# adobe/3D-FM-GAN

Hardware: AMD Instinct MI355X
Metric: (photo,render) pairs/sec (higher is better)
Workload: dtype f32; 1 GPU; pairs1024: cfg4 shard: E_Tsr+E_W+E_W_Plus(18 styles) on 256^2 -> co-mod -> Generator(1024) forward, fp32, B=8/GPU; pairs_per_gpu=8, global_pairs=8, image_size=1024, parallelism=replicas x1 (batch-sharded, no collective), launch=eager, ranks=1, full=False

## Files before the change

### 3d-fm-gan_amd/op/_native.py

```python
import ctypes
import os

import torch

_HERE = os.path.dirname(os.path.abspath(__file__))
LIB_PATH = os.environ.get('FMGAN_LIB') or os.path.join(os.path.dirname(_HERE), 'csrc', 'libfmgan_hip.so')

F32, F64, F16 = 0, 1, 2
FMGAN_OK, FMGAN_EUNSUPPORTED = 0, -2
LPIPS_SIZE = 256
_DTYPES = {torch.float32: F32, torch.float64: F64, torch.float16: F16}

_lib = None

amp_fwd = torch.amp.custom_fwd(device_type='cuda', cast_inputs=torch.float32)
amp_bwd = torch.amp.custom_bwd(device_type='cuda')


def _sig(fn, argtypes, restype=ctypes.c_int):
    fn.argtypes = argtypes
    fn.restype = restype
    return fn


def lib():
    global _lib
    if _lib is not None:
        return _lib
    if not os.path.exists(LIB_PATH):
        raise RuntimeError(
            f'{LIB_PATH} not found: the HIP extension is not built. Run `make -C {os.path.dirname(LIB_PATH)}` '
            f'(or __graft_entry__.build()). There is no CPU or PyTorch fallback for these ops.')
    L = ctypes.CDLL(LIB_PATH)
    vp, i, f, ll = ctypes.c_void_p, ctypes.c_int, ctypes.c_float, ctypes.c_longlong
    _sig(L.fmgan_abi_version, [])
    _sig(L.fmgan_status_string, [i], ctypes.c_char_p)
    _sig(L.fmgan_upfirdn2d_select, [i] * 15)
    _sig(L.fmgan_upfirdn2d_out_size, [i] * 12 + [ctypes.POINTER(i)] * 2)
    _sig(L.fmgan_upfirdn2d, [i, vp, vp, vp] + [i] * 15 + [vp])
    _sig(L.fmgan_upfirdn2d_strided, [i, vp, vp, vp] + [i] * 4 + [ll, i] + [i] * 11 + [vp])
    _sig(L.fmgan_blur_noise_bias_act_f32, [vp] * 3 + [i] * 4 + [ll, i] + [i] * 6 + [vp] * 3 + [i, f, f, vp])
    _sig(L.fmgan_blur_noise_bias_act_select, [vp] * 3 + [i] * 4 + [ll, i] + [i] * 6)
    _sig(L.fmgan_blur_noise_bias_act_path_f32, [vp] * 3 + [i] * 4 + [ll, i] + [i] * 6 + [vp] * 3 + [i, f, f, i, vp])
    _sig(L.fmgan_fused_bias_act, [i, vp, vp, vp, vp, ll, i, i, i, i, f, f, vp])
    _sig(L.fmgan_noise_bias_act_f32, [vp] * 5 + [i] * 4 + [f, f, vp])
    _sig(L.fmgan_fused_bias_act_bwd_blocks, [ll, i])
    _sig(L.fmgan_fused_bias_act_bwd_f32, [vp] * 4 + [ll, i, f, f, vp])
    _sig(L.fmgan_prelu_backward_blocks, [ll, i])
    _sig(L.fmgan_prelu_backward_f32, [vp] * 5 + [ll, i, vp])
    _sig(L.fmgan_face_region_blocks, [i, ll])
    _sig(L.fmgan_face_region_loss_f32, [vp] * 3 + [i, i, ll, vp])
    _sig(L.fmgan_face_region_backward_f32, [vp] * 4 + [i, i, ll, vp])
    _sig(L.fmgan_render_mask_f32, [vp] * 2 + [i, i, ll, vp])
    _sig(L.fmgan_face_input_blocks, [i] * 4)
    _sig(L.fmgan_face_input_f32, [vp] * 5 + [i] * 4 + [vp])
    _sig(L.fmgan_lpips_pair_input_select, [i] * 8)
    _sig(L.fmgan_lpips_pair_input_f32, [vp] * 5 + [i] * 8 + [vp])
    _sig(L.fmgan_projection_loss_select, [i] * 4)
    _sig(L.fmgan_projection_loss_blocks, [i] * 4)
    _sig(L.fmgan_projection_loss_fwd_f32, [vp] * 7 + [i] * 4 + [vp])
    _sig(L.fmgan_projection_loss_bwd_f32, [vp] * 7 + [i] * 4 + [vp])
    _sig(L.fmgan_fid_stats_select, [i] * 2)
    _sig(L.fmgan_fid_stats_update_f32, [vp] * 4 + [i, i, vp])
    _sig(L.fmgan_fid_stats_finish_f64, [vp] * 3 + [ll, vp, vp, i, vp])
    _sig(L.fmgan_inception_input_select, [i] * 3)
    _sig(L.fmgan_inception_input_f32, [vp, vp] + [i] * 4 + [vp])
    _sig(L.fmgan_lpips_distance_blocks, [i] * 3)
    _sig(L.fmgan_lpips_distance_f32, [vp] * 4 + [i, i, i, f, vp])
    _sig(L.fmgan_lpips_distance_backward_f32, [vp] * 6 + [i, i, i, f, vp])
    _sig(L.fmgan_bn_prelu_f32, [vp] * 5 + [f, vp, vp] + [vp] * 4 + [f, vp, vp] + [i] * 5 + [vp])
    _sig(L.fmgan_se_pool_chunks, [i] * 4)
    _sig(L.fmgan_se_pool_f32, [vp, vp] + [i] * 4 + [vp])
    _sig(L.fmgan_se_gate_f32, [vp, i, ll] + [vp] * 4 + [f] + [vp] * 3 + [i] * 3 + [vp])
    _sig(L.fmgan_ir_tail_f32, [vp] * 5 + [f, vp, vp] + [i] * 3 + [vp] * 4 + [f, vp] + [vp] * 4 + [f, vp] + [i] * 4 + [vp])
    _sig(L.fmgan_modconv_demod_f32, [vp] * 3 + [i] * 4 + [f, f, vp])
    _sig(L.fmgan_modconv_wsq_f32, [vp] * 2 + [i] * 3 + [vp])
    _sig(L.fmgan_modconv_demod_wsq_f32, [vp] * 3 + [i] * 3 + [f, f, vp])
    _sig(L.fmgan_equal_linear_f32, [vp] * 4 + [i] * 3 + [vp])
    _sig(L.fmgan_wino_weight_f32, [vp, vp, i, i, vp])
    _sig(L.fmgan_wino_input_f32, [vp] * 3 + [i] * 4 + [vp])
    _sig(L.fmgan_wino_output_f32, [vp] * 6 + [i] * 6 + [f, f, vp])
    _sig(L.fmgan_modconv_weight_prep_f32, [vp, vp, i, i, i, f, i, vp])
    _sig(L.fmgan_modconv2d_workspace_bytes, [i] * 6, ll)
    _sig(L.fmgan_modconv2d_f32, [vp] * 5 + [i] * 6 + [vp] * 3 + [i, i, f, f, ll, i, vp, ll, vp])
    _sig(L.fmgan_modconv_weight_bf16_bytes, [i] * 3, ll)
    _sig(L.fmgan_modconv_weight_to_bf16, [vp, vp, i, i, i, vp])
    _sig(L.fmgan_modconv2d_bf16_supported, [i] * 6)
    _sig(L.fmgan_modconv2d_bf16, [vp] * 5 + [i] * 6 + [vp] * 3 + [i, i, f, f, ll, i, vp])
    _sig(L.fmgan_modconv_weight_bf16x3_bytes, [i] * 3, ll)
    _sig(L.fmgan_modconv_weight_to_bf16x3, [vp, vp, i, i, i, vp])
    _sig(L.fmgan_modconv2d_bf16x3_supported, [i] * 6)
    _sig(L.fmgan_modconv2d_bf16x3, [vp] * 5 + [i] * 6 + [vp] * 3 + [i, i, f, f, ll, i, vp])
    _sig(L.fmgan_modconv2d_rgb_fusable, [i] * 5)
    _sig(L.fmgan_modconv2d_select, [i] * 8 + [ctypes.POINTER(i)] * 5)
    _sig(L.fmgan_modconv2d_tiles, [ctypes.POINTER(i), i])
    _sig(L.fmgan_torgb_weight_mod_f32, [vp] * 3 + [i] * 3 + [f, vp])
    _sig(L.fmgan_modconv2d_rgb_f32, [vp] * 5 + [i] * 5 + [vp] * 3 + [i, i, f, f] + [vp] * 4 + [i, vp])
    _sig(L.fmgan_modconv_wgrad_workspace_bytes, [i] * 5, ll)
    _sig(L.fmgan_modconv_wgrad_f32, [vp] * 5 + [i] * 5 + [f, vp, ll, vp])
    _sig(L.fmgan_modconv_wgrad_mode_workspace_bytes, [i] * 6, ll)
    _sig(L.fmgan_modconv_wgrad_mode_f32, [vp] * 5 + [i] * 6 + [f, vp, ll, vp])
    _sig(L.fmgan_images_to_tensor, [vp, vp, i, i, i, f, f, vp])
    _sig(L.fmgan_resize_output_size, [i, i, i, ctypes.POINTER(ctypes.c_int), ctypes.POINTER(ctypes.c_int)])
    _sig(L.fmgan_resize_plan_ints, [i] * 4, ll)
    _sig(L.fmgan_resize_plan, [i] * 4 + [vp, ll])
    _sig(L.fmgan_resize_bilinear_u8, [vp] * 4 + [i] * 5 + [f, f, vp])
    _sig(L.fmgan_tensor_to_images, [vp, vp, i, i, i, f, f, vp])
    _sig(L.fmgan_torgb_f32, [vp] * 6 + [i] * 4 + [f, vp])
    _sig(L.fmgan_torgb_backward_splits, [i] * 3)
    _sig(L.fmgan_torgb_backward_f32, [vp] * 6 + [i] * 4 + [f, vp])
    _sig(L.fmgan_refresh_entry_bytes, [])
    _sig(L.fmgan_weight_refresh_blocks, [i, i, i, i, ll], ll)
    _sig(L.fmgan_weight_refresh_f32, [vp, i, ll, vp])
    _sig(L.fmgan_style_bank_entry_bytes, [])
    _sig(L.fmgan_style_bank_f32, [vp, i, vp, vp, i, i, i, vp, vp])
    _sig(L.fmgan_demod_bank_f32, [vp, i, vp, i, vp, vp])
    if L.fmgan_abi_version() != 1:
        raise RuntimeError('libfmgan_hip.so ABI version mismatch')
    _lib = L
    return L


def check(status, what):
    if status != FMGAN_OK:
        raise RuntimeError(f'{what}: {lib().fmgan_status_string(status).decode()} (status {status})')


def served(status, what):
    if status == FMGAN_EUNSUPPORTED:
        return False
    check(status, what)
    return True


def require_gpu(t, name):
    if not t.is_cuda:
        raise RuntimeError(f'{name} must be a CUDA tensor (this build has no CPU path)')


def dtype_code(t):
    try:
        return _DTYPES[t.dtype]
    except KeyError:
        raise RuntimeError(f'unsupported dtype {t.dtype}: float32/float64/float16 only') from None


def ptr(t):
    return None if t is None else t.data_ptr()


def fp(t):
    if t is None:
        return None
    if t.dtype != torch.float32 or not t.is_cuda:
        raise RuntimeError(f'libfmgan_hip f32 entry point got a {t.dtype} tensor on {t.device}: float32 GPU tensors only '
                           f'(cast before the call; under autocast the package\'s autograd Functions do)')
    return t.data_ptr()


def require_f32_gpu(what, named, contiguous=True, same_device=True):
    first = None
    for t, name in named:
        if t is None:
            continue
        require_gpu(t, name)
        fp(t)
        if contiguous and not t.is_contiguous():
            raise RuntimeError(f'{what}: {name} must be contiguous, got strides {t.stride()}')
        if first is None:
            first = (t.device, name)
        elif same_device and t.device != first[0]:
            raise RuntimeError(f'{what}: {name} must be on {first[1]}\'s device')


class on_device:

    def __init__(self, t):
        self.dev = t.device
        self.guard = None

    def __enter__(self):
        if torch.cuda.current_device() != self.dev.index:
            self.guard = torch.cuda.device(self.dev)
            self.guard.__enter__()
        return torch.cuda.current_stream(self.dev).cuda_stream

    def __exit__(self, *exc):
        if self.guard is not None:
            self.guard.__exit__(*exc)
        return False


BLUR_PATHS = {}


class _NullObserver:
    wants_paths = False

    def begin(self, name, info):
        return None

    def end(self, token):
        pass


_observer = _NullObserver()


def set_observer(obs=None):
    global _observer
    _observer = obs if obs is not None else _NullObserver()


class launching(on_device):

    def __init__(self, t, name, info):
        on_device.__init__(self, t)
        self.name, self.info = name, info

    def __enter__(self):
        stream = on_device.__enter__(self)
        self.tok = _observer.begin(self.name, self.info)
        return stream

    def __exit__(self, *exc):
        if exc[0] is None:
            _observer.end(self.tok)
# ... 320 lines not shown

def projection_loss_bwd(x, target, mask, g_y, k, scale):
    b, h, w, f = _projection_loss_args(x, target, mask, (scale,))
    if k.numel() != 1 or k.device != x.device:
        raise ValueError(f'projection_loss_bwd: k must hold one element on x\'s device, got {tuple(k.shape)} on {k.device}')
    if g_y is not None:
        if tuple(g_y.shape) != (b, 3, LPIPS_SIZE, LPIPS_SIZE) or not nhwc_dense(g_y) or g_y.device != x.device:
            raise ValueError(f'projection_loss_bwd: g_y {tuple(g_y.shape)} with strides {g_y.stride()}: expected '
                             f'[{b}, 3, {LPIPS_SIZE}, {LPIPS_SIZE}] in channels_last storage on x\'s device')
    pk, pg = fp(k), fp(g_y)
    if b == 0 or lib().fmgan_projection_loss_select(b, h, w, f) <= 0:
        return None
    with launching(x, 'projection_loss', (b, h, f, mask is not None, g_y is not None, 1)) as stream:
        grad_x = torch.empty_like(x)
        st = lib().fmgan_projection_loss_bwd_f32(fp(x), fp(target), fp(mask), pg, pk, fp(scale), fp(grad_x), b, h, w, f,
                                                 stream)
    return grad_x if served(st, 'projection_loss_bwd') else None


def nhwc_dense(t):
    return t.ndim == 4 and t.permute(0, 2, 3, 1).is_contiguous()


def _lpips_distance_shape(f0, f1, w):
    if f0.ndim != 4 or tuple(f0.shape) != tuple(f1.shape) or w.numel() != f0.shape[1]:
        raise ValueError(f'lpips_distance: features {tuple(f0.shape)} and {tuple(f1.shape)}, weight {tuple(w.shape)}: '
                         f'expected two [N, C, H, W] tensors of one shape and C weights')
    if not (nhwc_dense(f0) and nhwc_dense(f1)):
        raise ValueError('lpips_distance: features must be NHWC-dense (channels_last storage); the kernel reads a '
                         'pixel\'s channel vector as one contiguous run')
    n, c, h, wd = f0.shape
    return n, c, h * wd


def lpips_distance(f0, f1, w, eps=1e-10):
    n, c, hw = _lpips_distance_shape(f0, f1, w)
    w = w.contiguous()
    p0, p1, pw = fp(f0), fp(f1), fp(w)
    if n == 0:
        return torch.zeros((0,), dtype=torch.float32, device=f0.device)
    blocks = lib().fmgan_lpips_distance_blocks(n, c, hw)
    if blocks <= 0:
        return None
    partial = torch.empty((n, blocks), dtype=torch.float32, device=f0.device)
    with launching(f0, 'lpips_distance', (n, c, hw, 0)) as stream:
        st = lib().fmgan_lpips_distance_f32(p0, p1, pw, fp(partial), n, c, hw, float(eps), stream)
    return partial.sum(1) / hw if served(st, 'lpips_distance') else None


def lpips_distance_backward(f0, f1, w, grad, need0, need1, eps=1e-10):
    n, c, hw = _lpips_distance_shape(f0, f1, w)
    if not (need0 or need1):
        return None, None
    gl = grad.reshape(-1)
    if gl.numel() != n:
        raise ValueError(f'lpips_distance_backward: grad must hold one element per sample ({n}), got {tuple(grad.shape)}')
    gl = gl.to(device=f0.device, dtype=torch.float32).contiguous()
    w = w.contiguous()
    p0, p1, pw, pg = fp(f0), fp(f1), fp(w), fp(gl)
    g0 = torch.empty_like(f0) if need0 else None
    g1 = torch.empty_like(f1) if need1 else None
    if n == 0:
        return g0, g1
    with launching(f0, 'lpips_distance', (n, c, hw, 1)) as stream:
        st = lib().fmgan_lpips_distance_backward_f32(p0, p1, pw, pg, fp(g0), fp(g1), n, c, hw, float(eps), stream)
    return (g0, g1) if served(st, 'lpips_distance_backward') else None


def _nhwc(t, name):
    require_gpu(t, name)
    fp(t)
    if not nhwc_dense(t):
        raise RuntimeError(f'{name}: expected a [B,C,H,W] tensor in channels_last storage, got {tuple(t.shape)} with '
                           f'strides {t.stride()}')
    return tuple(t.shape)


def _bn_args(bn, c):
    if bn is None:
        return None, None, None, None, 0.0
    mean, var, gamma, beta, eps = bn
    vs = [v.contiguous() for v in (mean, var, gamma, beta)]
    if any(v.numel() != c for v in vs):
        raise ValueError(f'BatchNorm vectors must hold {c} elements, got {[v.numel() for v in vs]}')
    return fp(vs[0]), fp(vs[1]), fp(vs[2]), fp(vs[3]), float(eps)


def _nhwc_empty(b, c, h, w, device):
    return torch.empty((b, c, h, w), dtype=torch.float32, device=device, memory_format=torch.channels_last)


def bn_prelu(x, bn, slope, want_y=True, bn_next=None, sub_stride=0):
    b, c, h, w = _nhwc(x, 'bn_prelu input')
    if not (want_y or bn_next is not None or sub_stride >= 1):
        raise ValueError('bn_prelu: no output requested')
    slope = slope.contiguous()
    if slope.numel() != c:
        raise ValueError(f'bn_prelu: {slope.numel()} slopes for {c} channels')
    y = torch.empty_like(x) if want_y else None
    y_next = torch.empty_like(x) if bn_next is not None else None
    y_sub = None
    if sub_stride >= 1:
        y_sub = _nhwc_empty(b, c, (h - 1) // sub_stride + 1, (w - 1) // sub_stride + 1, x.device)
    with launching(x, 'bn_prelu', (b, c, h, w)) as stream:
        st = lib().fmgan_bn_prelu_f32(fp(x), *_bn_args(bn, c), fp(slope), fp(y), *_bn_args(bn_next, c), fp(y_next),
                                      fp(y_sub), b, c, h, w, max(int(sub_stride), 0), stream)
    return (y, y_next, y_sub) if served(st, 'bn_prelu') else None


def se_pool(r):
    b, c, h, w = _nhwc(r, 'se_pool input')
    chunks = lib().fmgan_se_pool_chunks(b, c, h, w)
    if chunks <= 0:
        return None
    partial = torch.empty((b, chunks, c), dtype=torch.float32, device=r.device)
    with launching(r, 'se_pool', (b, c, h, w)) as stream:
        st = lib().fmgan_se_pool_f32(fp(r), fp(partial), b, c, h, w, stream)
    return partial if served(st, 'se_pool') else None


def se_gate(partial, hw, bn, fc1, fc2):
    require_gpu(partial, 'se_gate partials')
    b, chunks, c = partial.shape
    mid = fc1.shape[0]
    if tuple(fc1.shape[:2]) != (mid, c) or tuple(fc2.shape[:2]) != (c, mid) or fc1.numel() != mid * c \
            or fc2.numel() != mid * c:
        raise ValueError(f'se_gate: fc1 {tuple(fc1.shape)} / fc2 {tuple(fc2.shape)} do not fit {c} channels')
    fc1, fc2, partial = fc1.reshape(mid, c).contiguous(), fc2.reshape(c, mid).contiguous(), partial.contiguous()
    gate = torch.empty((b, c), dtype=torch.float32, device=partial.device)
    with launching(partial, 'se_gate', (b, c, mid, chunks)) as stream:
        st = lib().fmgan_se_gate_f32(fp(partial), chunks, int(hw), *_bn_args(bn, c), fp(fc1), fp(fc2), fp(gate), b, c,
                                     mid, stream)
    return gate if served(st, 'se_gate') else None


def ir_tail(r, bn, gate, shortcut, sc_stride=1, bn_sc=None, bn_next=None):
    b, c, h, w = _nhwc(r, 'ir_tail input')
    sb, scc, sh, sw = _nhwc(shortcut, 'ir_tail shortcut')
    exp = (h, w) if bn_sc is not None else ((sh - 1) // sc_stride + 1, (sw - 1) // sc_stride + 1)
    if (sb, scc) != (b, c) or exp != (h, w) or (bn_sc is not None and ((sh, sw) != (h, w) or sc_stride != 1)):
        raise ValueError(f'ir_tail: shortcut {tuple(shortcut.shape)} at stride {sc_stride} does not cover {tuple(r.shape)}')
    if gate is not None:
        if tuple(gate.shape) != (b, c):
            raise ValueError(f'ir_tail: gate {tuple(gate.shape)} for {tuple(r.shape)}')
        gate = gate.contiguous()
    out = torch.empty_like(r)
    out_next = torch.empty_like(r) if bn_next is not None else None
    with launching(r, 'ir_tail', (b, c, h, w, sc_stride, bn_sc is not None)) as stream:
        st = lib().fmgan_ir_tail_f32(fp(r), *_bn_args(bn, c), fp(gate), fp(shortcut), sh, sw, int(sc_stride),
                                     *_bn_args(bn_sc, c), fp(out), *_bn_args(bn_next, c), fp(out_next), b, c, h, w, stream)
    return (out, out_next) if served(st, 'ir_tail') else None


def modconv_demod(weight, style, scale, eps=1e-8, wsq=None):
    cout, cin, kh, kw = weight.shape[-4:]
    style = style.contiguous()
    demod = torch.empty((style.shape[0], cout), dtype=torch.float32, device=style.device)
    with on_device(style) as stream:
        if wsq is not None:
            check(lib().fmgan_modconv_demod_wsq_f32(fp(wsq), fp(style), fp(demod), style.shape[0], cout, cin,
                                                    float(scale), float(eps), stream), 'modconv_demod_wsq')
        else:
            check(lib().fmgan_modconv_demod_f32(fp(weight), fp(style), fp(demod), style.shape[0], cout, cin,
                                                kh * kw, float(scale), float(eps), stream), 'modconv_demod')
    return demod


def equal_linear(x, weight, bias=None):
    require_gpu(x, 'input')
    x, weight = x.contiguous(), weight.contiguous()
    b, k = x.shape
    n = weight.shape[0]
    if weight.shape[1] != k:
        raise RuntimeError(f'equal_linear: weight {tuple(weight.shape)} does not match input {tuple(x.shape)}')
    out = torch.empty((b, n), dtype=torch.float32, device=x.device)
    with on_device(x) as stream:
        check(lib().fmgan_equal_linear_f32(fp(x), fp(weight), fp(bias), fp(out), b, n, k, stream), 'equal_linear')
    return out


def style_bank(table, n_entries, w, wplus, styles_out):
    if w.dim() != 2 or wplus.dim() != 3 or wplus.shape[2] != w.shape[1] or not (w.is_contiguous() and wplus.is_contiguous()):
        raise RuntimeError(f'style_bank: W {tuple(w.shape)} / W+ {tuple(wplus.shape)} must be contiguous [T,D] / [P,n,D]')
    with on_device(w) as stream:
        check(lib().fmgan_style_bank_f32(fp(table.view(torch.float32)), n_entries, fp(w), fp(wplus), wplus.shape[0],
                                         w.shape[0], w.shape[1], fp(styles_out), stream), 'style_bank')


def demod_bank(table, n_entries, styles, batch, demod_out):
    with on_device(styles) as stream:
        check(lib().fmgan_demod_bank_f32(fp(table.view(torch.float32)), n_entries, fp(styles), batch, fp(demod_out), stream),
              'demod_bank')


def modconv_wsq(weight):
    cout, cin, kh, kw = weight.shape[-4:]
    wsq = torch.empty((cout, cin), dtype=torch.float32, device=weight.device)
    with on_device(weight) as stream:
        check(lib().fmgan_modconv_wsq_f32(fp(weight), fp(wsq), cout, cin, kh * kw, stream), 'modconv_wsq')
    return wsq


def modconv_weight_prep(weight, scale, kind=0):
    cout, cin, kh, kw = weight.shape[-4:]
    shape = (cin, kh * kw, cout) if kind == 0 else (cout, kh * kw, cin)
    wt = torch.empty(shape, dtype=torch.float32, device=weight.device)
    with on_device(weight) as stream:
        check(lib().fmgan_modconv_weight_prep_f32(fp(weight), fp(wt), cout, cin, kh * kw, float(scale), int(kind),
                                                  stream), 'modconv_weight_prep')
    return wt


def aligned_rows_shape(b, c, oh, ow, pad0):
    off = pad0 % 4
    rs = (ow + off + 31) // 32 * 32
    return (b * c, oh, rs), off, oh * rs, rs


def aligned_rows_buffer(b, c, oh, ow, pad0, device):
    shape, off, ps, rs = aligned_rows_shape(b, c, oh, ow, pad0)
    buf = torch.empty(shape, dtype=torch.float32, device=device)
    return buf, buf.data_ptr() + 4 * off, ps, rs


_mc_precision = 'f32'


class modconv_precision:

    def __init__(self, precision):
        if precision not in ('f32', 'bf16', 'bf16x3'):
            raise ValueError("precision must be 'f32', 'bf16' or 'bf16x3'")
        self.precision = precision

    def __enter__(self):
        global _mc_precision
        self.prev, _mc_precision = _mc_precision, self.precision
        return self

    def __exit__(self, *exc):
        global _mc_precision
        _mc_precision = self.prev
        return False


def modconv_weight_to_bf16(wt):
    cin, taps, cout = wt.shape
    nbytes = lib().fmgan_modconv_weight_bf16_bytes(cin, cout, taps)
    wtb = torch.empty(nbytes // 2, dtype=torch.int16, device=wt.device)
    with on_device(wt) as stream:
        check(lib().fmgan_modconv_weight_to_bf16(fp(wt), ptr(wtb), cin, cout, taps, stream), 'modconv_weight_to_bf16')
    return wtb


def wino_weight(wt):
    cin, taps, cout = wt.shape
    if taps != 9:
        raise RuntimeError('wino_weight: 3x3 weights only')
    u = torch.empty((16, cout, cin), dtype=torch.float32, device=wt.device)
    with on_device(wt) as stream:
        check(lib().fmgan_wino_weight_f32(fp(wt), fp(u), cin, cout, stream), 'wino_weight')
    return u


def wino_input(x, style):
    require_gpu(x, 'input')
    x, style = x.contiguous(), style.contiguous()
    b, cin, h, w = x.shape
    v = torch.empty((16, cin, b * (h // 2) * (w // 2)), dtype=torch.float32, device=x.device)
    with on_device(x) as stream:
        check(lib().fmgan_wino_input_f32(fp(x), fp(style), fp(v), b, cin, h, w, stream), 'wino_input')
    return v


def wino_output(m, demod, batch, h, w, noise=None, noise_weight=None, bias=None, fuse_act=False, alpha=0.2,
                act_scale=2 ** 0.5):
    require_gpu(m, 'm')
    m = m.contiguous()
    cout = m.shape[1]
    if m.shape[0] != 16 or m.shape[2] != batch * (h // 2) * (w // 2):
        raise RuntimeError('wino_output: M must be [16, cout, B*(H/2)*(W/2)]')
    out = torch.empty((batch, cout, h, w), dtype=torch.float32, device=m.device)
    nz, nb = _noise_args(noise)
    with on_device(m) as stream:
        check(lib().fmgan_wino_output_f32(fp(m), fp(demod), fp(nz), fp(noise_weight), fp(bias), fp(out), batch, cout, h, w,
                                          nb, int(bool(fuse_act)), float(alpha), float(act_scale), stream), 'wino_output')
    return out


def modconv2d_winograd(x, wt, style, demod, noise=None, noise_weight=None, bias=None, fuse_act=False, alpha=0.2,
                       act_scale=2 ** 0.5, u=None):
    require_gpu(x, 'input')
    x, style = x.contiguous(), style.contiguous()
    b, cin, h, w = x.shape
    if (h | w) & 1:
        raise RuntimeError('modconv2d_winograd: H and W must be even')
    if u is None:
        u = wino_weight(wt)
    cout = u.shape[1]
    n = b * (h // 2) * (w // 2)
    v = torch.empty((16, cin, n), dtype=torch.float32, device=x.device)
    m = torch.empty((16, cout, n), dtype=torch.float32, device=x.device)
    out = torch.empty((b, cout, h, w), dtype=torch.float32, device=x.device)
    nz, nb = _noise_args(noise)
    with launching(x, 'modconv2d_winograd', (b, cin, cout, h, w, 0)) as stream:
        check(lib().fmgan_wino_input_f32(fp(x), fp(style), fp(v), b, cin, h, w, stream), 'wino_input')
# ... 215 lines not shown
```

### 3d-fm-gan_amd/psp_encoder_model/encoders/psp_encoders.py

```python
import math
import os

import torch
import torch.nn.functional as F
from torch import nn
from torch.nn import BatchNorm2d, Conv2d, Module, Sequential

from . import helpers
from .helpers import PReLU, bottleneck_IR, bottleneck_IR_SE, get_blocks
from stylegan2 import EqualLinear
from op import fused_leaky_relu
from op.live_weights import LiveWeights
from Util.streams import overlap_ok, run_deferred, side_streams

HEAD_STREAMS = int(os.environ.get('FMGAN_PSP_STREAMS', '2'))
GROUP_HEADS = os.environ.get('FMGAN_PSP_GROUPED', '0') == '1'

_TAPS = {18: (3, 5, 7), 50: (6, 20, 23)}


class GradualStyleBlock(Module):

    def __init__(self, in_c, out_c, spatial):
        super().__init__()
        self.out_c = out_c
        self.spatial = spatial
        layers, c = [], in_c
        for _ in range(int(math.log2(spatial))):
            layers += [Conv2d(c, out_c, kernel_size=3, stride=2, padding=1), nn.LeakyReLU()]
            c = out_c
        self.convs = nn.Sequential(*layers)
        self.linear = EqualLinear(out_c, out_c, lr_mul=1)

    def forward(self, x):
        if x.is_cuda and x.dtype == torch.float32:
            for conv, act in zip(self.convs[0::2], self.convs[1::2]):
                y = F.conv2d(x, conv.weight, None, conv.stride, conv.padding)
                if y.is_contiguous(memory_format=torch.channels_last) and not y.is_contiguous():
                    n, c, h, w = y.shape
                    y = fused_leaky_relu(y.permute(0, 2, 3, 1).reshape(-1, c), conv.bias, act.negative_slope, 1.0)
                    x = y.view(n, h, w, c).permute(0, 3, 1, 2)
                else:
                    x = fused_leaky_relu(y, conv.bias, act.negative_slope, 1.0)
            return self.linear(x.reshape(-1, self.out_c))
        return self.linear(self.convs(x).reshape(-1, self.out_c))


class GradualStyleEncoder(Module):
    def __init__(self, num_layers, mode='ir', opts=None):
        super().__init__()
        assert num_layers in [18, 50, 100, 152], 'num_layers should be 18, 50, 100, or 152'
        assert mode in ['ir', 'ir_se'], 'mode should be ir or ir_se'
        self.num_layers = num_layers
        unit = bottleneck_IR if mode == 'ir' else bottleneck_IR_SE
        self.input_layer = Sequential(Conv2d(opts.input_nc, 64, (3, 3), 1, 1, bias=False), BatchNorm2d(64), PReLU(64))
        self.body = Sequential(*[unit(b.in_channel, b.depth, b.stride) for stage in get_blocks(num_layers) for b in stage])
        self.style_count = opts.n_styles
        self.coarse_ind = 3
        self.middle_ind = 7
        self.styles = nn.ModuleList()
        for i in range(self.style_count):
            spatial = 16 if i < self.coarse_ind else (32 if i < self.middle_ind else 64)
            self.styles.append(GradualStyleBlock(512, 512, spatial))
        self.latlayer1 = nn.Conv2d(256, 512, kernel_size=1, stride=1, padding=0)
        self.latlayer2 = nn.Conv2d(128, 512, kernel_size=1, stride=1, padding=0)
        self.channels_last = True
        self._cl_key = None
        self._live_weights = None
        self._flat = None

    def _to_channels_last(self):
        w = self.input_layer[0].weight
        key = (w.device, w.data_ptr())
        if self._cl_key != key:
            for m in self.modules():
                if isinstance(m, nn.Conv2d):
                    m.weight.data = m.weight.data.contiguous(memory_format=torch.channels_last)
            self._cl_key = (w.device, self.input_layer[0].weight.data_ptr())

    def _levels(self):
        n = self.style_count
        return [list(range(0, min(self.coarse_ind, n))), list(range(self.coarse_ind, min(self.middle_ind, n))),
                list(range(self.middle_ind, n))]

    def _flatten_heads(self):
        def aliased(big, parts):
            step = big[0:parts[0].shape[0]].numel() * big.element_size()
            return all(q.data_ptr() == big.data_ptr() + g * step and q.stride() == big[0:q.shape[0]].stride()
                       for g, q in enumerate(parts))
        if self._flat is not None and all(aliased(wb, [self.styles[j].convs[2 * d].weight for j in idxs]) and
                                          aliased(bb, [self.styles[j].convs[2 * d].bias for j in idxs])
                                          for idxs, per_depth in self._flat for d, (wb, bb) in enumerate(per_depth)):
            return self._flat
        flat = []
        with torch.no_grad():
            for idxs in self._levels():
                if not idxs:
                    continue
                per_depth = []
                for d in range(len(self.styles[idxs[0]].convs) // 2):
                    convs = [self.styles[j].convs[2 * d] for j in idxs]
                    wb = torch.cat([c.weight.data for c in convs], 0)
                    if convs[0].weight.data.is_contiguous(memory_format=torch.channels_last) and wb.dim() == 4:
                        wb = wb.contiguous(memory_format=torch.channels_last)
                    bb = torch.cat([c.bias.data for c in convs], 0)
                    co = convs[0].weight.shape[0]
                    for g, c in enumerate(convs):
                        c.weight.data = wb[g * co:(g + 1) * co]
                        c.bias.data = bb[g * co:(g + 1) * co]
                    per_depth.append((wb, bb))
                flat.append((idxs, per_depth))
        self._flat = flat
        return flat

    def _grouped_heads(self, level, feat):
        idxs, per_depth = level
        G = len(idxs)
        blocks = [self.styles[j] for j in idxs]
        x = feat
        for d, (wb, bb) in enumerate(per_depth):
            conv, act = blocks[0].convs[2 * d], blocks[0].convs[2 * d + 1]
            y = F.conv2d(x, wb, None, conv.stride, conv.padding, 1, 1 if d == 0 else G)
            n, c, h, w = y.shape
            if y.is_contiguous(memory_format=torch.channels_last) and not y.is_contiguous():
                y = fused_leaky_relu(y.permute(0, 2, 3, 1).reshape(-1, c), bb, act.negative_slope, 1.0)
                x = y.view(n, h, w, c).permute(0, 3, 1, 2)
            else:
                x = fused_leaky_relu(y, bb, act.negative_slope, 1.0)
        out_c = blocks[0].out_c
        xs = x.reshape(-1, G, out_c).transpose(0, 1)
        ws, bs = zip(*[b.linear._scaled_params() for b in blocks])
        out = torch.baddbmm(torch.stack(bs, 0).unsqueeze(1), xs, torch.stack(ws, 0).transpose(1, 2))
        return tuple(out.unbind(0))

    def _upsample_add(self, x, y):
        return F.interpolate(x, size=y.shape[2:], mode='bilinear', align_corners=True) + y

    def forward(self, x):
        heads = self.forward_deferred(x)
        for wait, _ in heads:
            wait()
        return torch.stack([t for _, t in heads], dim=1)

    def forward_deferred(self, x):
        if (not torch.is_grad_enabled()) and x.is_cuda:
            if self._live_weights is None:
                self._live_weights = LiveWeights(self)
            with self._live_weights.fresh():
                return self._forward_deferred(x)
        return self._forward_deferred(x)

    def _forward_deferred(self, x):
        if self.channels_last and x.is_cuda:
            self._to_channels_last()
            x = x.contiguous(memory_format=torch.channels_last)
        t1, t2, t3 = _TAPS[self.num_layers]
        fused = helpers.fused_body(self.input_layer, self.body, x, (t1, t2, t3))
        if fused is not None:
            x, feats = fused
        else:
            x = self.input_layer(x)
            feats = {}
            for i, unit in enumerate(self.body):
                x = unit(x)
                if i in (t1, t2, t3):
                    feats[i] = x
        c1, c2, c3 = feats[t1], feats[t2], feats[t3]
        if GROUP_HEADS and x.is_cuda and x.dtype == torch.float32 and not torch.is_grad_enabled():
            flat = self._flatten_heads()
            if HEAD_STREAMS > 1 and overlap_ok(x):
                streams = side_streams(x.device, HEAD_STREAMS, 'psp-heads')

                def level(k, feat):
                    wait, outs = run_deferred(streams[k % HEAD_STREAMS], self._grouped_heads, flat[k], feat)
                    return [(wait, o) for o in outs]
            else:
                def level(k, feat):
                    return [((lambda: None), o) for o in self._grouped_heads(flat[k], feat)]
            latents = level(0, c3)
            if len(flat) > 1:
                p2 = self._upsample_add(c3, self.latlayer1(c2))
                latents += level(1, p2)
            if len(flat) > 2:
                p1 = self._upsample_add(p2, self.latlayer2(c1))
                latents += level(2, p1)
            return latents
        if HEAD_STREAMS > 1 and overlap_ok(x):
            streams = side_streams(x.device, HEAD_STREAMS, 'psp-heads')

# ... 12 lines not shown
```

### include/fmgan_hip.h

```cpp
#ifndef FMGAN_HIP_H
#define FMGAN_HIP_H

#ifdef __cplusplus
extern "C" {
#endif

#define FMGAN_ABI_VERSION 1

#define FMGAN_OK            0
#define FMGAN_EINVAL       -1
#define FMGAN_EUNSUPPORTED -2
#define FMGAN_ELAUNCH      -3
#define FMGAN_EOVERFLOW    -4

#define FMGAN_F32 0
#define FMGAN_F64 1
#define FMGAN_F16 2

int         fmgan_abi_version(void);
const char *fmgan_status_string(int status);

int fmgan_upfirdn2d_select(int dtype, int major, int in_h, int in_w, int minor,
                           int kernel_h, int kernel_w, int up_x, int up_y,
                           int down_x, int down_y, int pad_x0, int pad_x1,
                           int pad_y0, int pad_y1);

int fmgan_upfirdn2d_out_size(int in_h, int in_w, int kernel_h, int kernel_w,
                             int up_x, int up_y, int down_x, int down_y,
                             int pad_x0, int pad_x1, int pad_y0, int pad_y1,
                             int *out_h, int *out_w);

int fmgan_upfirdn2d(int dtype, const void *input, const void *kernel, void *out,
                    int major, int in_h, int in_w, int minor,
                    int kernel_h, int kernel_w,
                    int up_x, int up_y, int down_x, int down_y,
                    int pad_x0, int pad_x1, int pad_y0, int pad_y1,
                    int force_path, void *stream);

int fmgan_upfirdn2d_strided(int dtype, const void *input, const void *kernel, void *out,
                            int major, int in_h, int in_w, int minor,
                            long long in_plane_stride, int in_row_stride,
                            int kernel_h, int kernel_w,
                            int up_x, int up_y, int down_x, int down_y,
                            int pad_x0, int pad_x1, int pad_y0, int pad_y1,
                            int force_path, void *stream);

int fmgan_blur_noise_bias_act_f32(const float *input, const float *kernel, float *out,
                                  int batch, int channels, int in_h, int in_w,
                                  long long in_plane_stride, int in_row_stride,
                                  int kernel_h, int kernel_w,
                                  int pad_x0, int pad_x1, int pad_y0, int pad_y1,
                                  const float *noise, const float *noise_weight, const float *bias,
                                  int noise_batch, float alpha, float act_scale, void *stream);
int fmgan_blur_noise_bias_act_select(const float *input, const float *out, const float *noise,
                                     int batch, int channels, int in_h, int in_w,
                                     long long in_plane_stride, int in_row_stride,
                                     int kernel_h, int kernel_w,
                                     int pad_x0, int pad_x1, int pad_y0, int pad_y1);
int fmgan_blur_noise_bias_act_path_f32(const float *input, const float *kernel, float *out,
                                       int batch, int channels, int in_h, int in_w,
                                       long long in_plane_stride, int in_row_stride,
                                       int kernel_h, int kernel_w,
                                       int pad_x0, int pad_x1, int pad_y0, int pad_y1,
                                       const float *noise, const float *noise_weight, const float *bias,
                                       int noise_batch, float alpha, float act_scale, int force_path, void *stream);

int fmgan_fused_bias_act(int dtype, const void *x, const void *bias, const void *refer,
                         void *out, long long size_x, int size_b, int step_b,
                         int act, int grad, float alpha, float scale, void *stream);

int fmgan_noise_bias_act_f32(const float *x, const float *noise, const float *noise_weight,
                             const float *bias, float *out,
                             int batch, int channel, int hw, int noise_batch,
                             float alpha, float scale, void *stream);

int fmgan_fused_bias_act_bwd_blocks(long long planes, int hw);
int fmgan_fused_bias_act_bwd_f32(const float *grad_out, const float *ref_out, float *grad_in, float *partial,
                                 long long planes, int hw, float alpha, float scale, void *stream);

int fmgan_prelu_backward_blocks(long long rows, int channels);
int fmgan_prelu_backward_f32(const float *x, const float *grad, const float *slope, float *grad_x,
                             float *partial, long long rows, int channels, void *stream);

int fmgan_face_region_blocks(int batch, long long hw);
int fmgan_face_region_loss_f32(const float *r, const float *g, float *partial, int batch, int channels, long long hw,
                               void *stream);
int fmgan_face_region_backward_f32(const float *r, const float *g, const float *grad_loss, float *grad_g, int batch,
                                   int channels, long long hw, void *stream);
int fmgan_render_mask_f32(const float *r, float *mask, int batch, int channels, long long hw, void *stream);

int fmgan_face_input_blocks(int batch, int h, int w, int k);
int fmgan_face_input_f32(const float *a, const float *b, float *gray_a, float *gray_b, float *l1_partial, int batch,
                         int h, int w, int k, void *stream);

int fmgan_lpips_pair_input_select(int pairs, int h, int w, int y0, int x0, int hc, int wc, int f);
int fmgan_lpips_pair_input_f32(const float *img, const float *shift, const float *scale, float *out0, float *out1,
                               int pairs, int h, int w, int y0, int x0, int hc, int wc, int f, void *stream);

int fmgan_projection_loss_select(int batch, int h, int w, int f);
int fmgan_projection_loss_blocks(int batch, int h, int w, int f);
int fmgan_projection_loss_fwd_f32(const float *x, const float *target, const float *mask, const float *shift,
                                  const float *scale, float *partial, float *y, int batch, int h, int w, int f,
                                  void *stream);
int fmgan_projection_loss_bwd_f32(const float *x, const float *target, const float *mask, const float *g_y,
                                  const float *k, const float *scale, float *grad_x, int batch, int h, int w, int f,
                                  void *stream);

int fmgan_fid_stats_select(int b, int d);
int fmgan_fid_stats_update_f32(const float *feat, const double *shift, double *sum, double *outer, int b, int d,
                               void *stream);
int fmgan_fid_stats_finish_f64(const double *sum, const double *outer, const double *shift, long long n, double *mean,
                               double *cov, int d, void *stream);

int fmgan_inception_input_select(int batch, int h, int w);
int fmgan_inception_input_f32(const float *img, float *out, int batch, int h, int w, int normalize, void *stream);

int fmgan_bn_prelu_f32(const float *x, const float *mean, const float *var, const float *gamma, const float *beta,
                       float eps, const float *slope, float *y, const float *next_mean, const float *next_var,
                       const float *next_gamma, const float *next_beta, float next_eps, float *y_next, float *y_sub,
                       int batch, int channels, int h, int w, int sub_stride, void *stream);
int fmgan_se_pool_chunks(int batch, int channels, int h, int w);
int fmgan_se_pool_f32(const float *r, float *partial, int batch, int channels, int h, int w, void *stream);
int fmgan_se_gate_f32(const float *partial, int chunks, long long hw, const float *mean, const float *var,
                      const float *gamma, const float *beta, float eps, const float *fc1, const float *fc2, float *gate,
                      int batch, int channels, int mid, void *stream);
int fmgan_ir_tail_f32(const float *r, const float *mean, const float *var, const float *gamma, const float *beta,
                      float eps, const float *gate, const float *shortcut, int sc_h, int sc_w, int sc_stride,
                      const float *sc_mean, const float *sc_var, const float *sc_gamma, const float *sc_beta, float sc_eps,
                      float *out, const float *next_mean, const float *next_var, const float *next_gamma,
                      const float *next_beta, float next_eps, float *out_next, int batch, int channels, int h, int w,
                      void *stream);

int fmgan_lpips_distance_blocks(int batch, int channels, int hw);
int fmgan_lpips_distance_f32(const float *f0, const float *f1, const float *w, float *partial, int batch, int channels,
                             int hw, float eps, void *stream);
int fmgan_lpips_distance_backward_f32(const float *f0, const float *f1, const float *w, const float *grad,
                                      float *grad_f0, float *grad_f1, int batch, int channels, int hw, float eps,
                                      void *stream);

int fmgan_modconv_demod_f32(const float *weight, const float *style, float *demod,
                            int batch, int cout, int cin, int ktaps,
                            float scale, float eps, void *stream);

int fmgan_wino_weight_f32(const float *wt, float *u, int cin, int cout, void *stream);
int fmgan_wino_input_f32(const float *x, const float *style, float *v, int batch, int c, int h, int w, void *stream);
int fmgan_wino_output_f32(const float *m, const float *demod, const float *noise, const float *noise_weight,
                          const float *bias, float *out, int batch, int cout, int h, int w, int noise_batch,
                          int fuse_act, float alpha, float act_scale, void *stream);

int fmgan_equal_linear_f32(const float *x, const float *weight, const float *bias, float *out,
                           int batch, int n_out, int k_in, void *stream);

int fmgan_modconv_wsq_f32(const float *weight, float *wsq, int cout, int cin, int ktaps, void *stream);
int fmgan_modconv_demod_wsq_f32(const float *wsq, const float *style, float *demod,
                                int batch, int cout, int cin, float scale, float eps, void *stream);

int fmgan_modconv_weight_prep_f32(const float *weight, float *wt, int cout, int cin, int ktaps,
                                  float scale, int kind, void *stream);

typedef struct fmgan_refresh_entry {
  const void *src;
  void *dst;
  void *dst2;
  long long n;
  int kind, cout, cin, ktaps;
  float scale;
  unsigned block_begin;
} fmgan_refresh_entry;
int fmgan_refresh_entry_bytes(void);
long long fmgan_weight_refresh_blocks(int kind, int cout, int cin, int ktaps, long long n);
int fmgan_weight_refresh_f32(const fmgan_refresh_entry *table_dev, int n_entries, long long total_blocks,
                             void *stream);

typedef struct fmgan_style_bank_entry {
  const void *ws;
  const void *bs;
  const void *wsq;
  long long style_off, demod_off;
  int col, sliced, n_styles, cin, cout, demodulate;
  float scale, eps;
} fmgan_style_bank_entry;
int fmgan_style_bank_entry_bytes(void);
int fmgan_style_bank_f32(const fmgan_style_bank_entry *table_dev, int n_entries, const float *w, const float *wplus,
                         int wplus_batch, int batch, int style_dim, float *styles_out, void *stream);
int fmgan_demod_bank_f32(const fmgan_style_bank_entry *table_dev, int n_entries, const float *styles, int batch,
                         float *demod_out, void *stream);

long long fmgan_modconv2d_workspace_bytes(int batch, int cin, int cout, int h, int w, int mode);
int fmgan_modconv2d_f32(const float *in, const float *wt, const float *style,
                        const float *demod, float *out,
                        int batch, int cin, int cout, int h, int w, int mode,
                        const float *noise, const float *noise_weight, const float *bias,
                        int noise_batch, int fuse_act, float alpha, float act_scale,
                        long long out_plane_stride, int out_row_stride,
                        void *workspace, long long workspace_bytes, void *stream);

long long fmgan_modconv_weight_bf16_bytes(int cin, int cout, int ktaps);
int fmgan_modconv_weight_to_bf16(const float *wt, void *wt_bf16, int cin, int cout, int ktaps, void *stream);
int fmgan_modconv2d_bf16_supported(int batch, int cin, int cout, int h, int w, int mode);
int fmgan_modconv2d_bf16(const float *in, const void *wt_bf16, const float *style, const float *demod, float *out,
                         int batch, int cin, int cout, int h, int w, int mode,
                         const float *noise, const float *noise_weight, const float *bias,
                         int noise_batch, int fuse_act, float alpha, float act_scale,
                         long long out_plane_stride, int out_row_stride, void *stream);

long long fmgan_modconv_weight_bf16x3_bytes(int cin, int cout, int ktaps);
int fmgan_modconv_weight_to_bf16x3(const float *wt, void *wt_split, int cin, int cout, int ktaps, void *stream);
int fmgan_modconv2d_bf16x3_supported(int batch, int cin, int cout, int h, int w, int mode);
int fmgan_modconv2d_bf16x3(const float *in, const void *wt_split, const float *style, const float *demod, float *out,
                           int batch, int cin, int cout, int h, int w, int mode,
                           const float *noise, const float *noise_weight, const float *bias,
                           int noise_batch, int fuse_act, float alpha, float act_scale,
                           long long out_plane_stride, int out_row_stride, void *stream);

int fmgan_torgb_weight_mod_f32(const float *rgb_weight, const float *rgb_style, float *wmod,
                               int batch, int cout, int rgb_channels, float rgb_scale, void *stream);
int fmgan_modconv2d_rgb_fusable(int batch, int cin, int cout, int h, int w);
int fmgan_modconv2d_rgb_f32(const float *in, const float *wt, const float *style,
                            const float *demod, float *out,
                            int batch, int cin, int cout, int h, int w,
                            const float *noise, const float *noise_weight, const float *bias,
                            int noise_batch, int fuse_act, float alpha, float act_scale,
                            const float *rgb_wmod, const float *rgb_bias,
                            const float *rgb_skip, float *rgb_out, int rgb_channels, void *stream);

int fmgan_modconv2d_select(int batch, int cin, int cout, int h, int w, int mode, int rgb, int has_workspace,
                           int *cfg, int *variant, int *bm, int *bn, int *ksplit);
int fmgan_modconv2d_tiles(int *out, int cap);

long long fmgan_modconv_wgrad_workspace_bytes(int batch, int cin, int cout, int h, int w);
long long fmgan_modconv_wgrad_mode_workspace_bytes(int batch, int cin, int cout, int h, int w, int mode);
int fmgan_modconv_wgrad_mode_f32(const float *go, const float *demod, const float *x, const float *style,
                                 float *gw, int batch, int cin, int cout, int h, int w, int mode, float scale,
                                 void *workspace, long long workspace_bytes, void *stream);
int fmgan_modconv_wgrad_f32(const float *go, const float *demod, const float *x, const float *style,
                            float *gw, int batch, int cin, int cout, int h, int w, float scale,
                            void *workspace, long long workspace_bytes, void *stream);

int fmgan_torgb_f32(const float *in, const float *weight, const float *style,
                    const float *bias, const float *skip, float *out,
                    int batch, int cin, int cout, int hw, float scale, void *stream);

int fmgan_torgb_backward_splits(int batch, int cin, int hw);
int fmgan_torgb_backward_f32(const float *x, const float *grad_out, const float *weight, const float *style,
                             float *grad_x, float *m_partial, int batch, int cin, int cout, int hw, float scale,
                             void *stream);

int fmgan_resize_output_size(int h, int w, int size, int *out_h, int *out_w);
long long fmgan_resize_plan_ints(int in_h, int in_w, int out_h, int out_w);
int fmgan_resize_plan(int in_h, int in_w, int out_h, int out_w, int *plan, long long plan_ints);
int fmgan_resize_bilinear_u8(const unsigned char *in, const int *plan, unsigned char *out_u8, float *out_f32,
                             int batch, int in_h, int in_w, int out_h, int out_w,
                             float mean, float stdv, void *stream);

int fmgan_images_to_tensor(const unsigned char *in, float *out, int batch, int h, int w,
                           float mean, float stdv, void *stream);
int fmgan_tensor_to_images(const float *in, unsigned char *out, int batch, int h, int w,
                           float cent, float factor, void *stream);

#ifdef __cplusplus
}
#endif
#endif
```

Before: 399.6 pairs/s.

## Add split-K MFMA kernel for small stride-2 pSp head convolutions

Adds a custom HIP kernel for the tail 3x3 stride-2 convolutions in the GradualStyleBlock heads at spatial size up to 4. It uses fp32 MFMA with split-K partials across blocks, then runs a finish kernel that sums the partials and fuses bias and leaky ReLU. The aim is to replace the poorly occupied library convolutions on tiny spatial maps, skip zero-padding taps at 1x1 outputs, and fold away the separate activation pass. It costs an extra workspace allocation and a second launch per conv, and it only runs in inference with grad disabled.

```diff
diff --git a/3d-fm-gan_amd/csrc/psp_head_tail.hip b/3d-fm-gan_amd/csrc/psp_head_tail.hip
--- /dev/null
+++ b/3d-fm-gan_amd/csrc/psp_head_tail.hip
@@ -0,0 +1,253 @@
+#include "common.h"
+
+namespace {
+
+constexpr int HC_CW = 2;
+constexpr int HC_KC4 = 8;
+constexpr int HC_MAX_M = 2048;
+
+struct HeadConvPlan {
+  int batch, h, cin, cout;
+  int m, ohw, ow;
+  int cin4;
+  unsigned cin4_rcp, nk_rcp;
+  int ohw_shift, ow_shift;
+  int k0, nk;
+  int k4;
+  int nchunks, cps, splits;
+  int mt, mchunks;
+  int cgroups;
+};
+
+typedef float f32x4acc __attribute__((ext_vector_type(4)));
+
+template <int MT>
+struct HeadConvOperands {
+  f32x4 w[2];
+  f32x4 x[MT][2];
+  unsigned wzero, xzero;
+};
+
+template <int MT>
+__global__ __launch_bounds__(256, 2) void head_conv_s2_partial(const float* __restrict__ x, const float* __restrict__ w,
+                                                            float* __restrict__ ws, const HeadConvPlan p) {
+  constexpr int CW = HC_CW, KW = 4 / HC_CW;
+  __shared__ float red[(KW > 1 ? (KW - 1) * CW * MT * 256 : 1)];
+  const int lane = threadIdx.x & 63, wave = threadIdx.x >> 6;
+  const int cw = wave % CW, kw = wave / CW;
+  const int i = lane & 15, g = lane >> 4;
+  const int o0 = (blockIdx.x * CW + cw) * 16;
+  const int o = o0 + i;
+  const bool o_ok = o < p.cout;
+  const float* wrow = w + (long long)(o_ok ? o : 0) * 9 * p.cin;
+  const int m0 = blockIdx.z * (MT * 16);
+
+  int base[MT], flag[MT];
+#pragma unroll
+  for (int t = 0; t < MT; ++t) {
+    const int m = m0 + t * 16 + i;
+    const int mm = m < p.m ? m : 0;
+    const int b = mm >> p.ohw_shift, r = mm - (b << p.ohw_shift);
+    const int oy = r >> p.ow_shift, ox = r - (oy << p.ow_shift);
+    base[t] = ((b * p.h + 2 * oy - 1) * p.h + 2 * ox - 1) * p.cin;
+    flag[t] = (oy == 0 ? 1 : 0) | (ox == 0 ? 2 : 0) | (m < p.m ? 0 : 4);
+  }
+
+  f32x4acc acc[MT];
+#pragma unroll
+  for (int t = 0; t < MT; ++t) acc[t] = f32x4acc{0.f, 0.f, 0.f, 0.f};
+
+  auto load = [&](int c, HeadConvOperands<MT>& v) {
+    int xoff[2], kflag[2];
+    v.wzero = v.xzero = 0;
+#pragma unroll
+    for (int hh = 0; hh < 2; ++hh) {
+      const int q = c * HC_KC4 + hh * 4 + g;
+      const bool k_ok = q < p.k4;
+      const int qq = k_ok ? q : 0;
+      const int tap = p.cin4 == 1 ? qq : (int)__umulhi(qq, p.cin4_rcp), ci = (qq - tap * p.cin4) * 4;
+      const int ty = __umulhi(tap, p.nk_rcp);
+      const int ky = p.k0 + ty, kx = p.k0 + tap - ty * p.nk;
+      v.w[hh] = *reinterpret_cast<const f32x4*>(wrow + (o_ok && k_ok ? (ky * 3 + kx) * p.cin + ci : 0));
+      v.wzero |= (o_ok && k_ok ? 0u : 1u) << hh;
+      xoff[hh] = (ky * p.h + kx) * p.cin + ci;
+      kflag[hh] = (ky == 0 ? 1 : 0) | (kx == 0 ? 2 : 0) | (k_ok ? 0 : 4);
+    }
+#pragma unroll
+    for (int t = 0; t < MT; ++t)
+#pragma unroll
+      for (int hh = 0; hh < 2; ++hh) {
+        const bool pad = (flag[t] & kflag[hh] & 3) != 0 || ((flag[t] | kflag[hh]) & 4) != 0;
+        v.x[t][hh] = *reinterpret_cast<const f32x4*>(x + (pad ? 0 : base[t] + xoff[hh]));
+        v.xzero |= (pad ? 1u : 0u) << (2 * t + hh);
+      }
+  };
+  auto mma = [&](const HeadConvOperands<MT>& v) {
+    const f32x4 zero = {0.f, 0.f, 0.f, 0.f};
+#pragma unroll
+    for (int hh = 0; hh < 2; ++hh) {
+      const f32x4 wv = (v.wzero >> hh) & 1 ? zero : v.w[hh];
+      f32x4 xv[MT];
+#pragma unroll
+      for (int t = 0; t < MT; ++t) xv[t] = (v.xzero >> (2 * t + hh)) & 1 ? zero : v.x[t][hh];
+#pragma unroll
+      for (int e = 0; e < 4; ++e)
+#pragma unroll
+        for (int t = 0; t < MT; ++t)
+          acc[t] = __builtin_amdgcn_mfma_f32_16x16x4f32(wv[e], xv[t][e], acc[t], 0, 0, 0);
+    }
+  };
+
+  const int c_begin = blockIdx.y * p.cps;
+  const int c_end = c_begin + p.cps < p.nchunks ? c_begin + p.cps : p.nchunks;
+  HeadConvOperands<MT> va, vb;
+  int c = c_begin + kw;
+  if (c < c_end) load(c, va);
+  for (; c < c_end; c += 2 * KW) {
+    const bool more = c + KW < c_end;
+    if (more) load(c + KW, vb);
+    mma(va);
+    if (more) {
+      if (c + 2 * KW < c_end) load(c + 2 * KW, va);
+      mma(vb);
+    }
+  }
+
+  if constexpr (KW > 1) {
+    if (kw > 0) {
+#pragma unroll
+      for (int t = 0; t < MT; ++t) {
+        float* dst = red + (((kw - 1) * CW + cw) * MT + t) * 256 + lane;
+        dst[0] = acc[t].x;
+        dst[64] = acc[t].y;
+        dst[128] = acc[t].z;
+        dst[192] = acc[t].w;
+      }
+    }
+    __syncthreads();
+  }
+  if (kw != 0) return;
+  const int ch = o0 + g * 4;
+#pragma unroll
+  for (int t = 0; t < MT; ++t) {
+    f32x4 v = {acc[t].x, acc[t].y, acc[t].z, acc[t].w};
+#pragma unroll
+    for (int k = 1; k < KW; ++k) {
+      const float* src = red + (((k - 1) * CW + cw) * MT + t) * 256 + lane;
+      v.x += src[0];
+      v.y += src[64];
+      v.z += src[128];
+      v.w += src[192];
+    }
+    const int m = m0 + t * 16 + i;
+    if (m < p.m && ch < p.cout)
+      *reinterpret_cast<f32x4*>(ws + ((long long)blockIdx.y * p.m + m) * p.cout + ch) = v;
+  }
+}
+
+__global__ __launch_bounds__(256) void head_conv_s2_finish(const float* __restrict__ ws, const float* __restrict__ bias,
+                                                           float* __restrict__ out, int n4, int cout4, int splits,
+                                                           float slope) {
+  const int idx = blockIdx.x * 256 + threadIdx.x;
+  if (idx >= n4) return;
+  const f32x4* p4 = reinterpret_cast<const f32x4*>(ws) + idx;
+  f32x4 s = p4[0];
+#pragma unroll 4
+  for (int k = 1; k < splits; ++k) {
+    const f32x4 v = p4[(long long)k * n4];
+    s.x += v.x;
+    s.y += v.y;
+    s.z += v.z;
+    s.w += v.w;
+  }
+  const f32x4 b = reinterpret_cast<const f32x4*>(bias)[idx % cout4];
+  f32x4 y;
+  y.x = s.x + b.x;
+  y.y = s.y + b.y;
+  y.z = s.z + b.z;
+  y.w = s.w + b.w;
+  y.x = y.x > 0.f ? y.x : y.x * slope;
+  y.y = y.y > 0.f ? y.y : y.y * slope;
+  y.z = y.z > 0.f ? y.z : y.z * slope;
+  y.w = y.w > 0.f ? y.w : y.w * slope;
+  reinterpret_cast<f32x4*>(out)[idx] = y;
+}
+
+unsigned rcp32(int d) { return (unsigned)((1ULL << 32) / (unsigned)d) + 1u; }
+
+int log2_exact(int v) {
+  int s = 0;
+  while ((1 << s) < v) ++s;
+  return s;
+}
+
+int head_conv_plan(int batch, int h, int w, int cin, int cout, HeadConvPlan* p) {
+  if (batch <= 0 || h <= 0 || w <= 0 || cin <= 0 || cout <= 0) return FMGAN_EINVAL;
+  if (h != w || (h != 2 && h != 4 && h != 8 && h != 16)) return FMGAN_EUNSUPPORTED;
+  if (cin % 4 != 0 || cout % 4 != 0 || cin > 4096 || cout > 4096) return FMGAN_EUNSUPPORTED;
+  const int oh = h / 2;
+  if ((long long)batch * oh * oh > HC_MAX_M) return FMGAN_EUNSUPPORTED;
+  p->batch = batch, p->h = h, p->cin = cin, p->cout = cout;
+  p->ohw = oh * oh, p->ow = oh, p->m = batch * oh * oh;
+  p->cin4 = cin / 4;
+  p->ohw_shift = log2_exact(p->ohw), p->ow_shift = log2_exact(p->ow);
+  p->k0 = oh > 1 ? 0 : 1;
+  p->nk = 3 - p->k0;
+  p->k4 = p->nk * p->nk * p->cin4;
+  p->cin4_rcp = rcp32(p->cin4), p->nk_rcp = rcp32(p->nk);
+  p->nchunks = (p->k4 + HC_KC4 - 1) / HC_KC4;
+  p->mt = p->m <= 16 ? 1 : p->m <= 32 ? 2 : p->m <= 64 ? 4 : 8;
+  p->mchunks = (p->m + p->mt * 16 - 1) / (p->mt * 16);
+  const int ctiles = (cout + 15) / 16;
+  p->cgroups = (ctiles + HC_CW - 1) / HC_CW;
+  int splits = (256 + p->cgroups * p->mchunks - 1) / (p->cgroups * p->mchunks);
+  if (splits > p->nchunks / (4 / HC_CW)) splits = p->nchunks / (4 / HC_CW);
+  if (splits < 1) splits = 1;
+  p->cps = (p->nchunks + splits - 1) / splits;
+  p->splits = (p->nchunks + p->cps - 1) / p->cps;
+  return FMGAN_OK;
+}
+
+bool aligned16(const void* q) { return (reinterpret_cast<uintptr_t>(q) & 15) == 0; }
+
+}
+
+extern "C" int fmgan_head_conv_s2_select(int batch, int h, int w, int cin, int cout, int* tiles, int* splits, int* taps) {
+  HeadConvPlan p;
+  const int st = head_conv_plan(batch, h, w, cin, cout, &p);
+  if (st != FMGAN_OK) return st;
+  if (tiles) *tiles = p.mt;
+  if (splits) *splits = p.splits;
+  if (taps) *taps = p.nk * p.nk;
+  return 1;
+}
+
+extern "C" long long fmgan_head_conv_s2_workspace_bytes(int batch, int h, int w, int cin, int cout) {
+  HeadConvPlan p;
+  if (head_conv_plan(batch, h, w, cin, cout, &p) != FMGAN_OK) return 0;
+  return (long long)p.splits * p.m * p.cout * 4;
+}
+
+extern "C" int fmgan_head_conv_s2_f32(const float* x, const float* w, const float* bias, float* out, float* workspace,
+                                      long long workspace_bytes, int batch, int h, int wd, int cin, int cout,
+                                      float slope, void* stream) {
+  HeadConvPlan p;
+  const int st = head_conv_plan(batch, h, wd, cin, cout, &p);
+  if (st != FMGAN_OK) return st;
+  if (!x || !w || !bias || !out || !workspace) return FMGAN_EINVAL;
+  if (workspace_bytes < (long long)p.splits * p.m * p.cout * 4) return FMGAN_EINVAL;
+  if (!aligned16(x) || !aligned16(w) || !aligned16(bias) || !aligned16(out) || !aligned16(workspace))
+    return FMGAN_EUNSUPPORTED;
+  hipStream_t s = (hipStream_t)stream;
+  const dim3 grid(p.cgroups, p.splits, p.mchunks);
+  switch (p.mt) {
+    case 1: hipLaunchKernelGGL(head_conv_s2_partial<1>, grid, dim3(256), 0, s, x, w, workspace, p); break;
+    case 2: hipLaunchKernelGGL(head_conv_s2_partial<2>, grid, dim3(256), 0, s, x, w, workspace, p); break;
+    case 4: hipLaunchKernelGGL(head_conv_s2_partial<4>, grid, dim3(256), 0, s, x, w, workspace, p); break;
+    default: hipLaunchKernelGGL(head_conv_s2_partial<8>, grid, dim3(256), 0, s, x, w, workspace, p); break;
+  }
+  const int n4 = p.m * (p.cout / 4);
+  hipLaunchKernelGGL(head_conv_s2_finish, dim3((n4 + 255) / 256), dim3(256), 0, s, workspace, bias, out, n4, p.cout / 4,
+                     p.splits, slope);
+  return fmgan_check_launch();
+}
diff --git a/3d-fm-gan_amd/op/_native.py b/3d-fm-gan_amd/op/_native.py
--- a/3d-fm-gan_amd/op/_native.py
+++ b/3d-fm-gan_amd/op/_native.py
@@ -73,6 +73,9 @@
     _sig(L.fmgan_se_pool_f32, [vp, vp] + [i] * 4 + [vp])
     _sig(L.fmgan_se_gate_f32, [vp, i, ll] + [vp] * 4 + [f] + [vp] * 3 + [i] * 3 + [vp])
     _sig(L.fmgan_ir_tail_f32, [vp] * 5 + [f, vp, vp] + [i] * 3 + [vp] * 4 + [f, vp] + [vp] * 4 + [f, vp] + [i] * 4 + [vp])
+    _sig(L.fmgan_head_conv_s2_select, [i] * 5 + [ctypes.POINTER(i)] * 3)
+    _sig(L.fmgan_head_conv_s2_workspace_bytes, [i] * 5, ll)
+    _sig(L.fmgan_head_conv_s2_f32, [vp] * 5 + [ll] + [i] * 5 + [f, vp])
     _sig(L.fmgan_modconv_demod_f32, [vp] * 3 + [i] * 4 + [f, f, vp])
     _sig(L.fmgan_modconv_wsq_f32, [vp] * 2 + [i] * 3 + [vp])
     _sig(L.fmgan_modconv_demod_wsq_f32, [vp] * 3 + [i] * 3 + [f, f, vp])
@@ -699,6 +702,36 @@
     return (out, out_next) if served(st, 'ir_tail') else None
 
 
+def head_conv_s2_select(x, weight):
+    if x.dim() != 4 or weight.dim() != 4 or tuple(weight.shape[1:]) != (x.shape[1], 3, 3) or x.shape[0] == 0:
+        return None
+    if not (nhwc_dense(x) and nhwc_dense(weight)):
+        return None
+    b, cin, h, w = x.shape
+    v = [ctypes.c_int() for _ in range(3)]
+    st = lib().fmgan_head_conv_s2_select(b, h, w, cin, weight.shape[0], *[ctypes.byref(c) for c in v])
+    return tuple(c.value for c in v) if st > 0 else None
+
+
+def head_conv_s2(x, weight, bias, slope):
+    require_gpu(x, 'input')
+    if head_conv_s2_select(x, weight) is None:
+        return None
+    bias = bias.contiguous()
+    b, cin, h, w = x.shape
+    cout = weight.shape[0]
+    if bias.numel() != cout:
+        raise ValueError(f'head_conv_s2: {bias.numel()} bias values for {cout} channels')
+    require_f32_gpu('head_conv_s2', ((x, 'input'), (weight, 'weight'), (bias, 'bias')), contiguous=False)
+    ws_bytes = lib().fmgan_head_conv_s2_workspace_bytes(b, h, w, cin, cout)
+    with launching(x, 'head_conv_s2', (b, cin, cout, h)) as stream:
+        out = _nhwc_empty(b, cout, h // 2, w // 2, x.device)
+        ws = torch.empty(ws_bytes // 4, dtype=torch.float32, device=x.device)
+        st = lib().fmgan_head_conv_s2_f32(fp(x), fp(weight), fp(bias), fp(out), fp(ws), ws_bytes, b, h, w, cin, cout,
+                                          float(slope), stream)
+    return out if served(st, 'head_conv_s2') else None
+
+
 def modconv_demod(weight, style, scale, eps=1e-8, wsq=None):
     cout, cin, kh, kw = weight.shape[-4:]
     style = style.contiguous()
diff --git a/3d-fm-gan_amd/psp_encoder_model/encoders/psp_encoders.py b/3d-fm-gan_amd/psp_encoder_model/encoders/psp_encoders.py
--- a/3d-fm-gan_amd/psp_encoder_model/encoders/psp_encoders.py
+++ b/3d-fm-gan_amd/psp_encoder_model/encoders/psp_encoders.py
@@ -9,14 +9,21 @@
 from . import helpers
 from .helpers import PReLU, bottleneck_IR, bottleneck_IR_SE, get_blocks
 from stylegan2 import EqualLinear
-from op import fused_leaky_relu
+from op import _native, fused_leaky_relu
 from op.live_weights import LiveWeights
 from Util.streams import overlap_ok, run_deferred, side_streams
 
 HEAD_STREAMS = int(os.environ.get('FMGAN_PSP_STREAMS', '2'))
 GROUP_HEADS = os.environ.get('FMGAN_PSP_GROUPED', '0') == '1'
+HEAD_TAILS = os.environ.get('FMGAN_NO_HEAD_TAILS', '0') != '1'
+HEAD_TAIL_MAX = int(os.environ.get('FMGAN_HEAD_TAIL_MAX', '4'))
 
 _TAPS = {18: (3, 5, 7), 50: (6, 20, 23)}
+
+
+def _is_tail_conv(conv):
+    return (conv.kernel_size == (3, 3) and conv.stride == (2, 2) and conv.padding == (1, 1) and conv.dilation == (1, 1)
+            and conv.groups == 1 and conv.padding_mode == 'zeros' and conv.bias is not None)
 
 
 class GradualStyleBlock(Module):
@@ -34,7 +41,13 @@
 
     def forward(self, x):
         if x.is_cuda and x.dtype == torch.float32:
+            tails = HEAD_TAILS and not torch.is_grad_enabled() and not torch.is_autocast_enabled()
             for conv, act in zip(self.convs[0::2], self.convs[1::2]):
+                if tails and x.shape[2] <= HEAD_TAIL_MAX and _is_tail_conv(conv):
+                    y = _native.head_conv_s2(x, conv.weight, conv.bias, act.negative_slope)
+                    if y is not None:
+                        x = y
+                        continue
                 y = F.conv2d(x, conv.weight, None, conv.stride, conv.padding)
                 if y.is_contiguous(memory_format=torch.channels_last) and not y.is_contiguous():
                     n, c, h, w = y.shape
diff --git a/include/fmgan_hip.h b/include/fmgan_hip.h
--- a/include/fmgan_hip.h
+++ b/include/fmgan_hip.h
@@ -131,6 +131,12 @@
                       const float *next_beta, float next_eps, float *out_next, int batch, int channels, int h, int w,
                       void *stream);
 
+int fmgan_head_conv_s2_select(int batch, int h, int w, int cin, int cout, int *tiles, int *splits, int *taps);
+long long fmgan_head_conv_s2_workspace_bytes(int batch, int h, int w, int cin, int cout);
+int fmgan_head_conv_s2_f32(const float *x, const float *w, const float *bias, float *out, float *workspace,
+                           long long workspace_bytes, int batch, int h, int wd, int cin, int cout, float slope,
+                           void *stream);
+
 int fmgan_lpips_distance_blocks(int batch, int channels, int hw);
 int fmgan_lpips_distance_f32(const float *f0, const float *f1, const float *w, float *partial, int batch, int channels,
                              int hw, float eps, void *stream);
```

Measured after the change: 398.0 pairs/s. About the same (-0.4%).
